# Yeicor/sdf-viewer

Hardware: AMD Instinct MI355X
Metric: Mvoxels/s grid fill + Mrays/s sphere-trace @1080p, demo SDF (higher is better)
Workload: dtype f32

## Files before the change

### include/sdfgrid.h

```cpp
#ifndef SDFGRID_H
#define SDFGRID_H

#include <stddef.h>
#include <stdint.h>

#ifdef __cplusplus
extern "C" {
#endif

#define SDFV_ABI_VERSION 5

typedef enum sdfv_status {
    SDFV_OK = 0,
    SDFV_ERR_INVALID_ARGUMENT = -1,
    SDFV_ERR_UNKNOWN_SDF = -2,
    SDFV_ERR_HIP = -3,
    SDFV_ERR_NO_DEVICE = -4,
    SDFV_ERR_COMM = -5
} sdfv_status;

typedef struct sdfv_sample {
    float distance;
    float color[3];
    float metallic;
// ... 58 lines not shown
    int32_t status;
    int32_t steps;
    float   hit_pos[3];
    float   t;
    float   raw0[4];
    float   raw1[4];
    float   normal[3];
    float   depth;
} sdfv_march_aux;

uint32_t    sdfv_abi_version(void);
const char *sdfv_last_error(void);
const char *sdfv_build_id(void);
int         sdfv_device_count(void);
float       sdfv_air_dist(void);

typedef enum sdfv_option {
    SDFV_OPT_FILL_NONTEMPORAL = 1,
    SDFV_OPT_FILL_FORM = 2,
    SDFV_OPT_RAYMARCH_DISABLE = 3,
    SDFV_OPT_RAYMARCH_KEEP_NORMAL = 4,
    SDFV_OPT_SLAB_STEP_FORM = 5,
    SDFV_OPT_RAYMARCH_TILE_GROUP = 6,
    SDFV_OPT_RAYMARCH_BOX_FIRST = 7,
    SDFV_OPT_RAYMARCH_WAVES_PER_SIMD = 8,
    SDFV_OPT_RAYMARCH_BATCH_STREAMS = 9,
    SDFV_OPT_EXT_SRGB_QUANT = 10,
    SDFV_OPT_PASS_INDEX_LIMIT = 11,
    SDFV_OPT_RAYMARCH_CAMERA_STAGING = 12,
    SDFV_OPT_PASS_FORM = 13,
    SDFV_OPT_PASS_LOADS = 15,
    SDFV_OPT_RCCL_LIBRARY = 14,
    SDFV_OPT_RAYMARCH_LOD_FILTER = 16,
    SDFV_OPT_TUNING_WAVE_TIMING = 100,
    SDFV_OPT_TUNING_TILE_ORDER = 102,
    SDFV_OPT_TUNING_PRIORITY_MAP = 101
} sdfv_option;
#define SDFV_RM_NO_FAST_INDEX  1u
#define SDFV_RM_NO_POW2_EXTENT 2u
#define SDFV_RM_NO_POW2_SIZE   4u
#define SDFV_RM_NO_SYMMETRIC   8u
#define SDFV_RM_NO_ASM_LOOP   16u
#define SDFV_RM_NO_INTERIOR_FETCH 32u
#define SDFV_STEP_SIDE_BOUNDARY 3u
#define SDFV_STEP_UNPACKED     4u
#define SDFV_STEP_START_EVENT  8u
#define SDFV_STEP_DEFER_JOIN  16u
int sdfv_set_option(uint32_t option, uint64_t value);
int sdfv_get_option(uint32_t option, uint64_t *value);

void sdfv_demo_params_default(sdfv_demo_params *p);
int  sdfv_grid_from_bb(const float bb_min[3], const float bb_max[3], uint32_t max_voxels_side, sdfv_grid *out);
void sdfv_render_params_default(sdfv_render_params *rp, const sdfv_grid *grid);
int  sdfv_camera_look_at(sdfv_camera *cam, const float eye[3], const float target[3], const float up[3],
                         float fovy_degrees, float aspect, float z_near, float z_far);


int sdfv_grid_init(const sdfv_grid *grid, float *tex0, float *tex1, void *stream);

int sdfv_grid_init_unvisited(const sdfv_grid *grid, uint32_t step, float *tex0, float *tex1, float *dist, void *stream);
int sdfv_grid_init_unvisited_ex(const sdfv_grid *grid, uint32_t step, float *tex0, float *tex1, float *dist, uint32_t flags,
                                void *stream);

int sdfv_fill_grid(const sdfv_demo_params *params, uint32_t sdf_id, const sdfv_grid *grid,
                   float *tex0, float *tex1, void *stream);

// ... 311 lines not shown
```

### sdf-viewer_amd/_capi.py

```python
import ctypes as C
import os

_HERE = os.path.dirname(os.path.abspath(__file__))
LIB_PATH = os.environ.get("SDFGRID_LIBRARY") or os.path.join(_HERE, "libsdfgrid.so")


class SdfvError(RuntimeError):
    def __init__(self, code, message):
        super().__init__(f"libsdfgrid error {code}: {message}")
        self.code = code


class Sample(C.Structure):
    _fields_ = [("distance", C.c_float), ("color", C.c_float * 3), ("metallic", C.c_float),
                ("roughness", C.c_float), ("occlusion", C.c_float)]


class DemoParams(C.Structure):
    _fields_ = [("cube_half_side", C.c_float), ("cube_material", C.c_uint32),
                ("sphere_radius", C.c_float), ("sphere_material", C.c_uint32),
                ("max_distance_custom_material", C.c_float), ("disable_sphere", C.c_uint32)]


class Grid(C.Structure):
# ... 171 lines not shown
                                            C.c_uint32, C.POINTER(Mesh), C.c_void_p]),
    "sdfv_lattice_normals": (C.c_int, [C.c_void_p, C.POINTER(C.c_float), C.POINTER(C.c_float), C.c_uint32, C.c_void_p, C.c_size_t,
                                       C.c_void_p]),
}
MESH_WITH_MATERIALS = 1
MESHER_MARCHING_CUBES = 0
MESHER_DUAL_CONTOURING_PARTICLE = 4
LIGHT_AMBIENT, LIGHT_DIRECTIONAL, MAX_LIGHTS = 0, 1, 4


def raymarch_rc(rp, tex0, tex1, cameras, n_cameras, width, height, y0, y1, rgba, depth=None, aux=None, dist=None, pairs=None,
                ilv=None, band_first=0, band_step=0, stream=None, size=None, band_height=0):
    d = MarchDesc()
    d.size = C.sizeof(d) if size is None else size
    d.rp = C.pointer(rp) if rp is not None else None
    d.tex0, d.tex1, d.dist, d.pairs, d.ilv = tex0, tex1, dist, pairs, ilv
    if cameras is not None:
        d.cameras = C.cast(C.pointer(cameras), C.POINTER(Camera))
    d.n_cameras, d.width, d.height, d.y0, d.y1 = n_cameras, width, height, y0, y1
    d.band_first, d.band_step, d.band_height = band_first, band_step, band_height
    d.rgba, d.depth, d.aux = rgba, depth, aux
    return lib.sdfv_raymarch_ex(C.byref(d), stream)
OPT_FILL_NONTEMPORAL, OPT_FILL_FORM, OPT_RAYMARCH_DISABLE, OPT_RAYMARCH_KEEP_NORMAL, OPT_SLAB_STEP_FORM = 1, 2, 3, 4, 5
OPT_RAYMARCH_TILE_GROUP = 6
OPT_RAYMARCH_BOX_FIRST = 7
OPT_RAYMARCH_WAVES_PER_SIMD = 8
OPT_RAYMARCH_BATCH_STREAMS = 9
OPT_PASS_INDEX_LIMIT = 11
OPT_RAYMARCH_CAMERA_STAGING = 12
OPT_PASS_FORM = 13
OPT_RCCL_LIBRARY = 14
OPT_PASS_LOADS = 15
OPT_RAYMARCH_LOD_FILTER = 16
OPT_EXT_SRGB_QUANT = 10
OPT_TUNING_WAVE_TIMING = 100
OPT_TUNING_PRIORITY_MAP = 101
OPT_TUNING_TILE_ORDER = 102
RM_NO_FAST_INDEX, RM_NO_POW2_EXTENT, RM_NO_POW2_SIZE, RM_NO_SYMMETRIC, RM_NO_ASM_LOOP, RM_NO_INTERIOR_FETCH = 1, 2, 4, 8, 16, 32
STEP_SIDE_BOUNDARY, STEP_UNPACKED, STEP_START_EVENT, STEP_DEFER_JOIN = 3, 4, 8, 16
PASS_FRESH_GRID, PASS_SAME_LOAD, PASS_VIRGIN_GRID, PASS_VOLUME_INTERLEAVED, PASS_EXPECT_NOOP = 1, 2, 4, 8, 16
(OP_SPHERE, OP_CUBE, OP_BOX, OP_CYLINDER, OP_TORUS, OP_PLANE, OP_PUSH_AFFINE, OP_PUSH_SCALE, OP_POP, OP_POP_SCALE, OP_UNION,
 OP_INTERSECT, OP_SUBTRACT, OP_SMOOTH_UNION, OP_SMOOTH_SUBTRACT, OP_ROUND, OP_SHELL, OP_MATERIAL) = range(1, 19)
PROGRAM_MAX_OPS, PROGRAM_MAX_VALUES, PROGRAM_MAX_FRAMES = 256, 8, 4
FILL_FORM = {"auto": 0, "rows": 1, "flat": 2}
COMM_ID_BYTES = 128
RAY_BUFFER_HEADER_BYTES = 16
MARCH_MERGE = 1
COMM_PERIODIC = 1
COMM_HALO2 = 2


def load(path=LIB_PATH):
    if not os.path.exists(path):
        raise ImportError(
            f"{path} not found: build it with `python -c 'import __graft_entry__ as g; g.build()'` "
            "(or `make -C sdf-viewer_amd/csrc`).  There is no CPU fallback.")
    lib = C.CDLL(path)
    for name, (restype, argtypes) in PROTOTYPES.items():
        fn = getattr(lib, name)
        fn.restype = restype
        fn.argtypes = argtypes
    return lib


lib = load()

# ... 9 lines not shown
```

### sdf-viewer_amd/csrc/api_common.hip

```cpp
#include <atomic>
#include <cmath>
#include <cstdarg>
#include <cstdio>
#include <cstring>
#include <mutex>
#include <string>

#include "api_internal.h"

namespace sdfv {
thread_local char g_err[512] = "";
thread_local Options g_options;

int set_error(int code, const char* fmt, ...) {
    va_list ap;
    va_start(ap, fmt);
    vsnprintf(g_err, sizeof(g_err), fmt, ap);
    va_end(ap);
    return code;
}

int hip_fail(hipError_t e, const char* what) {
    if (e == hipErrorNoDevice || e == hipErrorInvalidDevice)
        return set_error(SDFV_ERR_NO_DEVICE, "%s: no HIP device (%s)", what, hipGetErrorString(e));
// ... 112 lines not shown

int sdfv_set_option(uint32_t option, uint64_t value) {
    auto out_of_range = [&] {
        return set_error(SDFV_ERR_INVALID_ARGUMENT, "value %llu is out of range for option %u", (unsigned long long)value, option);
    };
    for (const auto& o : kPlainOptions) {
        if (o.option != option) continue;
        if (value > o.max) return out_of_range();
        g_options.*o.member = (uint32_t)value;
        return SDFV_OK;
    }
    switch (option) {
        case SDFV_OPT_SLAB_STEP_FORM: {
            const uint64_t form = value & ~(uint64_t)(SDFV_STEP_UNPACKED | SDFV_STEP_START_EVENT | SDFV_STEP_DEFER_JOIN);
            if (form != 0 && form != SDFV_STEP_SIDE_BOUNDARY) break;
            g_options.slab_step_form = (uint32_t)value;
            return SDFV_OK;
        }
        case SDFV_OPT_PASS_INDEX_LIMIT:
            if (value != 0 && (value < 2 || value > (1ull << 32))) break;
            g_options.pass_index_limit = value;
            return SDFV_OK;
        case SDFV_OPT_RCCL_LIBRARY: {
            const char* path = reinterpret_cast<const char*>((uintptr_t)value);
            if (path && strnlen(path, 4096) >= 4096) break;
            if (!sdfv::set_rccl_library_path(path))
                return set_error(SDFV_ERR_INVALID_ARGUMENT, "SDFV_OPT_RCCL_LIBRARY: RCCL has already been loaded in this process");
            return SDFV_OK;
        }
        case SDFV_OPT_RAYMARCH_WAVES_PER_SIMD:
            if (value == 1 || value > 7) break;
            g_options.raymarch_waves_per_simd = (uint32_t)value;
            return SDFV_OK;
        case SDFV_OPT_TUNING_TILE_ORDER: case SDFV_OPT_TUNING_PRIORITY_MAP: case SDFV_OPT_TUNING_WAVE_TIMING: {
#ifdef SDFV_TUNING
            (option == SDFV_OPT_TUNING_TILE_ORDER ? g_options.tile_order
             : option == SDFV_OPT_TUNING_PRIORITY_MAP ? g_options.priority_map : g_options.wave_timing) = value;
            return SDFV_OK;
#else
            const char* name = option == SDFV_OPT_TUNING_TILE_ORDER ? "TILE_ORDER" : option == SDFV_OPT_TUNING_PRIORITY_MAP ? "PRIORITY_MAP" : "WAVE_TIMING";
            return set_error(SDFV_ERR_INVALID_ARGUMENT, "SDFV_OPT_TUNING_%s needs the tuning build (make tuning)", name);
#endif
        }
        default:
            return set_error(SDFV_ERR_INVALID_ARGUMENT, "unknown option %u", option);
    }
    return out_of_range();
}

int sdfv_get_option(uint32_t option, uint64_t* value) {
    if (!value) return set_error(SDFV_ERR_INVALID_ARGUMENT, "value is NULL");
    for (const auto& o : kPlainOptions)
        if (o.option == option) {
            *value = g_options.*o.member;
            return SDFV_OK;
        }
    switch (option) {
        case SDFV_OPT_SLAB_STEP_FORM: *value = g_options.slab_step_form; return SDFV_OK;
        case SDFV_OPT_TUNING_WAVE_TIMING: *value = g_options.wave_timing; return SDFV_OK;
        case SDFV_OPT_TUNING_PRIORITY_MAP: *value = g_options.priority_map; return SDFV_OK;
        case SDFV_OPT_TUNING_TILE_ORDER: *value = g_options.tile_order; return SDFV_OK;
        case SDFV_OPT_RAYMARCH_WAVES_PER_SIMD: *value = g_options.raymarch_waves_per_simd; return SDFV_OK;
        case SDFV_OPT_PASS_INDEX_LIMIT: *value = g_options.pass_index_limit; return SDFV_OK;
        case SDFV_OPT_RCCL_LIBRARY: {
            thread_local std::string copy;
            copy = sdfv::rccl_library_path_copy();
            *value = (uint64_t)(uintptr_t)copy.c_str();
            return SDFV_OK;
        }
        default: return set_error(SDFV_ERR_INVALID_ARGUMENT, "unknown option %u", option);
    }
}

void sdfv_demo_params_default(sdfv_demo_params* p) {
    if (!p) return;
    p->cube_half_side = 0.95f;
    p->cube_material = SDFV_MATERIAL_BRICK;
    p->sphere_radius = 1.05f;
    p->sphere_material = SDFV_MATERIAL_NORMAL;
    p->max_distance_custom_material = 0.05f;
    p->disable_sphere = 0;
}

int sdfv_grid_from_bb(const float bb_min[3], const float bb_max[3], uint32_t max_voxels_side, sdfv_grid* out) {
    if (!bb_min || !bb_max || !out) return set_error(SDFV_ERR_INVALID_ARGUMENT, "NULL argument");
    float size[3] = {bb_max[0] - bb_min[0], bb_max[1] - bb_min[1], bb_max[2] - bb_min[2]};
    int max_dim = 0;
    for (int i = 1; i < 3; ++i)
        if (size[i] >= size[max_dim]) max_dim = i;
    for (int i = 0; i < 3; ++i) {
        if (i == max_dim) {
            out->dims[i] = max_voxels_side;
        } else {
            float v = (float)max_voxels_side * size[i] / size[max_dim];
            out->dims[i] = v > 0.0f ? (uint32_t)v : 0u;
// ... 53 lines not shown
```

### sdf-viewer_amd/csrc/api_internal.h

```cpp
#pragma once

#include <hip/hip_runtime.h>

#include <cstdint>
#include <cstring>
#include <string>

#include "../../include/sdfgrid.h"

namespace sdfv {
struct Options {
    uint32_t fill_nontemporal = 0;
    uint32_t fill_form = 0;
    uint32_t raymarch_disable = 0;
    uint32_t raymarch_keep_normal = 0;
    uint32_t raymarch_lod_filter = 0;
    uint32_t raymarch_batch_streams = 1;
    uint32_t raymarch_camera_staging = 1;
    uint32_t raymarch_box_first = 1;
    uint32_t raymarch_waves_per_simd = 0;
    uint32_t raymarch_tile_group = 0;
    uint32_t slab_step_form = 0;
    uint32_t ext_srgb_quant = 0;
    uint32_t pass_form = 0;
    uint32_t pass_loads = 0;
    unsigned long long pass_index_limit = 0;
    unsigned long long wave_timing = 0;
    unsigned long long priority_map = 0;
    unsigned long long tile_order = 0;
};
extern thread_local char g_err[512];
extern thread_local Options g_options;
inline const Options& options() { return g_options; }
std::string rccl_library_path_copy();
const char* claim_rccl_library_path();
int set_error(int code, const char* fmt, ...) __attribute__((format(printf, 2, 3)));
int hip_fail(hipError_t e, const char* what);
#define SDFV_HIP(call)                                          \
    do {                                                        \
        hipError_t e_ = (call);                                 \
        if (e_ != hipSuccess) return sdfv::hip_fail(e_, #call); \
    } while (0)
#define SDFV_HIP_RETURN(call) return sdfv::hip_status((call), #call)
inline int hip_status(hipError_t e, const char* what) { return e == hipSuccess ? SDFV_OK : hip_fail(e, what); }

int check_params(const sdfv_demo_params* p, uint32_t sdf_id);
int check_grid(const sdfv_grid* g);
int check_lights(const sdfv_render_params* rp);
int need_device();
inline int need_textures(const void* tex0, const void* tex1) {
    return tex0 && tex1 ? SDFV_OK : set_error(SDFV_ERR_INVALID_ARGUMENT, "texture pointer is NULL");
}
template <typename... P>
// ... 96 lines not shown
```

### sdf-viewer_amd/csrc/api_march.hip

```cpp
#include <cmath>
#include <cstddef>
#include <cstring>

#include "api_internal.h"
#include "march_common.h"
#include "raymarch_kernels.h"

using namespace sdfv;

namespace {

struct BatchStreams {
    static constexpr int kSide = 3;
    hipStream_t side[kSide] = {};
    hipEvent_t fork = nullptr, join[kSide] = {};
    int device = -1;
    void release() {
        for (int i = 0; i < kSide; ++i) {
            if (side[i]) (void)hipStreamDestroy(side[i]);
            if (join[i]) (void)hipEventDestroy(join[i]);
        }
        if (fork) (void)hipEventDestroy(fork);
        *this = BatchStreams{};
    }
// ... 118 lines not shown
    if (int rc = check_lights(rp)) return rc;
    if (int rc = check_texel_alignment(d.tex0, d.tex1, d.rgba)) return rc;
    if (int rc = check_word_aligned("dist, depth, aux and rgba8", d.dist, d.depth, d.aux, d.rgba8)) return rc;
    if (((uintptr_t)d.pairs | (uintptr_t)d.ilv) & 7) return set_error(SDFV_ERR_INVALID_ARGUMENT, "pairs and ilv must be 8-byte aligned");
    if (n_cameras && !cameras) return set_error(SDFV_ERR_INVALID_ARGUMENT, "cameras is NULL");
    if (y0 > y1 || y1 > height) return set_error(SDFV_ERR_INVALID_ARGUMENT, "rows [%u,%u) outside height %u", y0, y1, height);
    if (rp->tex_size[0] == 0 || rp->tex_size[1] == 0 || rp->tex_size[2] == 0)
        return set_error(SDFV_ERR_INVALID_ARGUMENT, "empty texture");
    if (!(rp->lod_dist_between_samples >= 1.0f)) return set_error(SDFV_ERR_INVALID_ARGUMENT, "lod_dist_between_samples < 1");
    const uint32_t lod_filter = g_options.raymarch_lod_filter;
    if (lod_filter == 1 && rp->lod_dist_between_samples != 1.0f) {
        int e = 0;
        const float lod = rp->lod_dist_between_samples;
        if (!(lod >= 2.0f && lod <= 32768.0f) || frexpf(lod, &e) != 0.5f)
            return set_error(SDFV_ERR_INVALID_ARGUMENT,
                             "SDFV_OPT_RAYMARCH_LOD_FILTER 1: lod_dist_between_samples %g is not a power of two in [2, 32768]", (double)lod);
    }
    if ((uint64_t)rp->tex_size[0] * rp->tex_size[1] * rp->tex_size[2] >= (1ull << 32))
        return set_error(SDFV_ERR_INVALID_ARGUMENT, "texture too large for 32-bit texel indexing");
    if (int rc = need_device()) return rc;
    sdfv::RaymarchArgs a;
    derive_raymarch_args(rp, a);
    a.dist = d.dist;
    a.pairs = d.pairs;
    a.ilv = d.ilv;
    set_march_frame(a, d.tex0, d.tex1, width, height, y0, y1);
    a.band_skip = band_height * (band_step - 1u);
    a.band_shift = band_height == 8u ? 3u : 4u;
    a.rows_out = band_step > 1 ? sdfv_band_rows_ex(height, y0 / band_height, band_step, band_height) : y1 - y0;
    a.compute_normal = g_options.raymarch_keep_normal ? 1u : 0u;
    const uint32_t w = g_options.raymarch_waves_per_simd;
    a.waves_per_simd = w;
    a.box_first = g_options.raymarch_box_first;
    const DeviceFacts& dev = device_facts();
    if (!dev.gfx950) a.asm_loop = 0;
    a.wave_slots_per_simd_unit = dev.cus * 4u;
    a.last_level_cache_bytes = dev.last_level_cache_bytes;
    const bool xcd_order_ok = dev.xcds == 8;
    a.group_shift = g_options.raymarch_tile_group == 0 ? (n_cameras == 1 && xcd_order_ok ? sdfv::kGroupAuto : 0u)
                                                       : (g_options.raymarch_tile_group == 1 ? 0u : g_options.raymarch_tile_group - 1u);
    a.rotate_columns = g_options.raymarch_tile_group == 0 && xcd_order_ok ? 1u : 0u;
#ifdef SDFV_TUNING
    a.wave_timing = reinterpret_cast<unsigned long long*>(g_options.wave_timing);
    a.priority_map = reinterpret_cast<const unsigned char*>(g_options.priority_map);
    a.tile_order = n_cameras == 1 ? reinterpret_cast<const uint32_t*>(g_options.tile_order) : nullptr;
#endif
    const uint64_t pixels_per_cam = (uint64_t)a.rows_out * width;
    hipStream_t main = (hipStream_t)stream;
    const sdfv_camera* device_cameras = nullptr;
    bool ring = false;
    hipPointerAttribute_t attr;
    if (hipPointerGetAttributes(&attr, cameras) == hipSuccess && (attr.type == hipMemoryTypeDevice || attr.type == hipMemoryTypeManaged)) {
        device_cameras = cameras;
    } else {
        (void)hipGetLastError();
        if (n_cameras > sdfv::kInlineCameras) {
            hipStreamCaptureStatus capturing = hipStreamCaptureStatusNone;
            if (hipStreamIsCapturing(main, &capturing) != hipSuccess) (void)hipGetLastError();
            ring = capturing == hipStreamCaptureStatusNone && g_options.raymarch_camera_staging &&
                   g_camera_ring.ensure(current_device()) == hipSuccess;
        }
    }
    const uint32_t per_launch = device_cameras || ring ? sdfv::kMaxCamerasPerLaunch : sdfv::kInlineCameras;
    const uint64_t groups_per_launch = (uint64_t)((width + 15) / 16) * ((a.rows_out + 15) / 16) * per_launch;
    const bool overlap = n_cameras > per_launch && groups_per_launch <= 40000 && g_options.raymarch_batch_streams;
    uint32_t used = 0;
// ... 217 lines not shown
```

### sdf-viewer_amd/csrc/march_common.h

```cpp
#pragma once

#include "march_shade.h"

#if defined(__HIPCC__)
#define SDFV_MARCH_FN __device__ __forceinline__
#define SDFV_MARCH_HD __host__ __device__ __forceinline__
#else
#define SDFV_MARCH_FN inline
#define SDFV_MARCH_HD inline
#endif

namespace sdfv {
namespace march {

struct V3 {
    float x, y, z;
};
SDFV_MARCH_FN V3 mk(float x, float y, float z) { V3 r; r.x = x; r.y = y; r.z = z; return r; }
SDFV_MARCH_FN V3 sub(V3 a, V3 b) { return mk(a.x - b.x, a.y - b.y, a.z - b.z); }
SDFV_MARCH_FN V3 madd(V3 a, V3 d, float t) { return mk(a.x + d.x * t, a.y + d.y * t, a.z + d.z * t); }
SDFV_MARCH_FN float length(V3 a) { return sqrtf(a.x * a.x + a.y * a.y + a.z * a.z); }
SDFV_MARCH_FN V3 normalize(V3 a) {
    const float l = length(a);
    return mk(a.x / l, a.y / l, a.z / l);
// ... 42 lines not shown
}
SDFV_MARCH_FN V3 tap_sign(int t) { return mk((t == 0 || t == 3) ? 1.0f : -1.0f, t >= 2 ? 1.0f : -1.0f, (t & 1) ? 1.0f : -1.0f); }
SDFV_MARCH_FN V3 normal_tap(V3 p, float h, int t) {
    const V3 k = tap_sign(t);
    return mk(p.x + k.x * h, p.y + k.y * h, p.z + k.z * h);
}
SDFV_MARCH_FN V3 normal_of_taps(float d1, float d2, float d3, float d4) {
    return normalize(mk(d1 + -d2 + -d3 + d4, -d1 + -d2 + d3 + d4, -d1 + d2 + -d3 + d4));
}

SDFV_MARCH_FN void aux_clear(sdfv_march_aux& aux) {
    aux.status = 0; aux.steps = 0;
    aux.hit_pos[0] = aux.hit_pos[1] = aux.hit_pos[2] = 0.0f;
    aux.t = 0.0f;
    aux.raw0[0] = aux.raw0[1] = aux.raw0[2] = aux.raw0[3] = 0.0f;
    aux.raw1[0] = aux.raw1[1] = aux.raw1[2] = aux.raw1[3] = 0.0f;
    aux.normal[0] = aux.normal[1] = aux.normal[2] = 0.0f;
    aux.depth = 1.0f;
}
SDFV_MARCH_FN void aux_set_march(sdfv_march_aux& aux, int status, int steps, V3 ray_pos, float dist_from_origin) {
    aux.status = status;
    aux.steps = steps;
    aux.hit_pos[0] = ray_pos.x; aux.hit_pos[1] = ray_pos.y; aux.hit_pos[2] = ray_pos.z;
    aux.t = dist_from_origin;
}
SDFV_MARCH_FN void aux_set_hit(sdfv_march_aux& aux, float4 raw0, float4 raw1, V3 n, float depth) {
    aux.raw0[0] = raw0.x; aux.raw0[1] = raw0.y; aux.raw0[2] = raw0.z; aux.raw0[3] = raw0.w;
    aux.raw1[0] = raw1.x; aux.raw1[1] = raw1.y; aux.raw1[2] = raw1.z; aux.raw1[3] = raw1.w;
    aux.normal[0] = n.x; aux.normal[1] = n.y; aux.normal[2] = n.z;
    aux.depth = depth;
}

#if defined(__HIPCC__)
SDFV_MARCH_FN void tile_pixel(uint32_t bx, uint32_t by, uint32_t& px, uint32_t& row) {
    const uint32_t lane = threadIdx.x & 63, wave = threadIdx.x >> 6;
    px = bx * 16 + (wave & 1) * 8 + (lane & 7);
    row = by * 16 + (wave >> 1) * 8 + (lane >> 3);
}

template <typename Args>
SDFV_MARCH_FN void store_color(const Args& a, uint64_t out_index, float4 v) {
    typedef float v4f __attribute__((ext_vector_type(4)));
    if (a.rgba) {
        const v4f t = {v.x, v.y, v.z, v.w};
        __builtin_nontemporal_store(t, reinterpret_cast<v4f*>(a.rgba + out_index));
    }
    if (a.rgba8) __builtin_nontemporal_store(rgba_unorm8(v), a.rgba8 + out_index);
}
#endif

}
}
```

### sdf-viewer_amd/csrc/program_march_kernels.hip

```cpp
#include "program_march_kernels.h"

#include "kernel_common.h"

namespace sdfv {

namespace {

template <bool AUX>
__device__ __forceinline__ void program_march(const ProgramMarchArgs& a) {
    __shared__ float s_lut[256];
    const LdsLut lut = stage_srgb_lut(s_lut);
    __syncthreads();

    uint32_t px, row;
    march::tile_pixel(blockIdx.x, blockIdx.y, px, row);
    const uint32_t py = a.y0 + row;
    const uint32_t cam_idx = blockIdx.z;
    const bool in_image = px < a.f.width && py < a.y1;
    const sdfv_camera& cam = a.cameras[cam_idx];
    const uint64_t out_index = ((uint64_t)cam_idx * (a.y1 - a.y0) + row) * a.f.width + px;

    float4 rgba;
    sdfv_march_aux aux;
    pmarch::march_pixel_program(a.f, cam, px, py, in_image, lut, rgba, aux);
    if (!in_image) return;
    march::store_color(a, out_index, rgba);
    if (a.depth) a.depth[out_index] = aux.depth;
    if (AUX) a.aux[out_index] = aux;
}

}

extern "C" {

__global__ __launch_bounds__(kBlock) void sdfprog_march(ProgramMarchArgs a) { program_march<false>(a); }
__global__ __launch_bounds__(kBlock) void sdfprog_march_aux(ProgramMarchArgs a) { program_march<true>(a); }

}

hipError_t launch_program_march(const ProgramMarchArgs& a, hipStream_t stream) {
    if (a.f.width == 0 || a.y1 <= a.y0 || a.n_cameras == 0) return hipSuccess;
    if (a.n_cameras > kProgramMarchCameras) return hipErrorInvalidValue;
    const uint32_t tiles_x = (a.f.width + 15) / 16, tiles_y = (a.y1 - a.y0 + 15) / 16;
    if (tiles_y > 65535u) return hipErrorInvalidValue;
    hipLaunchKernelGGL(a.aux ? sdfprog_march_aux : sdfprog_march, dim3(tiles_x, tiles_y, a.n_cameras), dim3(kBlock), 0, stream, a);
    return hipGetLastError();
}

// ... 2 lines not shown
```

### sdf-viewer_amd/csrc/raymarch_kernels.h

```cpp
#pragma once

#include <hip/hip_runtime.h>
#include <stdint.h>

#include "../../include/sdfgrid.h"

namespace sdfv {

struct RaymarchArgs {
    sdfv_render_params rp;
    float bsize[3];
    float inv_bsize[3];
    uint32_t pow2_extent;
    uint32_t fast_index;
    const float* dist;
    const float* pairs;
    const float* ilv;
    uint32_t pow2_size;
    uint32_t symmetric_box;
    uint32_t fast_normal;
    float cull_center[3];
    float cull_radius2;
    const float4* tex0;
    const float4* tex1;
    uint32_t n_cameras;
    uint32_t width, height;
    uint32_t y0, y1;
    uint32_t compute_normal;
    uint32_t asm_loop;
    uint32_t group_shift;
    uint32_t tiles_x, tiles_y, groups_x;
    uint32_t box_first;
    uint32_t first_gx0, first_gy0, first_w, first_h, m_groups_x, m_first_w, m_rest_w;
    uint32_t no_interior_fetch;
    uint32_t rotate_columns;
    uint32_t lds_cap_bytes;
    uint32_t waves_per_simd;
    uint32_t wave_slots_per_simd_unit;
    uint64_t last_level_cache_bytes;
    uint32_t cube_box;
    uint32_t rows_out;
    uint32_t band_skip;
    uint32_t band_shift;
    float4* rgba;
    uint32_t* rgba8;
    sdfv_march_aux* aux;
    float* depth;
#ifdef SDFV_TUNING
    const uint32_t* tile_order;
    const unsigned char* priority_map;
    unsigned long long* wave_timing;
#endif
    const sdfv_camera* camera_list;
    sdfv_camera cameras[16];
};

constexpr int kMarchGeneral = 0, kMarchTex0 = 1, kMarchDist = 2, kMarchPairs = 3, kMarchIlv = 4, kMarchLattice = 5;

constexpr uint32_t kInlineCameras = 16;
constexpr uint32_t kMaxCamerasPerLaunch = 64;
constexpr uint32_t kGroupAuto = 255;

struct SlabMarchArgs {
    uint32_t z_lo, z_count;
    uint32_t own_begin, own_end;
    const sdfv_ray_state* in;
    uint32_t n_in;
    const uint32_t* in_count[2];
    const sdfv_ray_state* in_rays[2];
    uint32_t max_in;
// ... 17 lines not shown
```

### sdf-viewer_amd/csrc/raymarch_kernels.hip

```cpp
#include "raymarch_kernels.h"

#include <hip/hip_runtime.h>
#include <string.h>

#include "march_common.h"

namespace sdfv {
namespace {

using namespace march;

__device__ __forceinline__ uint32_t mirror_index(int i, int n) {
    if (i >= 0 && i < n) return (uint32_t)i;
    int period = 2 * n;
    int m = i % period;
    if (m < 0) m += period;
    return (uint32_t)(m < n ? m : period - 1 - m);
}

struct Tex {
    const float4* data;
    int w, h, d;
    int z_lo;
};
// ... 546 lines not shown
#define SDFV_MARCH_ASM_PER_VOLUME(RUN)                                                                              \
    if (MODE == kMarchIlv) { SDFV_MARCH_ASM_PER_BOX(RUN, SDFV_MARCH_ASM_VOL_ILV); }                                 \
    else if (MODE == kMarchPairs) { SDFV_MARCH_ASM_PER_BOX(RUN, SDFV_MARCH_ASM_VOL_PAIRS); }                        \
    else if (MODE == kMarchDist) { SDFV_MARCH_ASM_PER_BOX(RUN, SDFV_MARCH_ASM_VOL_DIST); }                          \
    else { SDFV_MARCH_ASM_PER_BOX(RUN, SDFV_MARCH_ASM_VOL_TEX0); }
    const bool cube = a.cube_box != 0;
    if (T) {
        float tt = dist_from_origin;
        int n = 0;
        SDFV_MARCH_ASM_PER_VOLUME(SDFV_MARCH_ASM_RUN_AUX)
        dist_from_origin = tt;
        steps = n;
    } else {
        SDFV_MARCH_ASM_PER_VOLUME(SDFV_MARCH_ASM_RUN)
    }
#ifdef SDFV_TUNING
    iterations = cov ? (min(255, 255 - (int)(short)(left & 0xffff)) | (left & 0xffff0000)) : 0;
#else
    (void)iterations;
    (void)left;
#endif
    if (covered) {
        ray_pos = mk(px, py, pz);
        const bool ran = ((ran_out >> (threadIdx.x & 63)) & 1ull) != 0;
        status = ran ? -1 : (oob_dist<true>(a, ray_pos) > 1e-4f ? -2 : 1);
    }
}

#ifdef SDFV_TUNING
__device__ __forceinline__ void stamp_wave(const RaymarchArgs& a, uint32_t bx, uint32_t by, uint32_t wave,
                                           unsigned long long t_start, unsigned long long t_start_rt, int iterations,
                                           unsigned long long covered_mask) {
    const uint32_t tiles_x = (a.width + 15) / 16, tiles_y = (a.rows_out + 15) / 16;
    const uint64_t wave_id = ((uint64_t)(blockIdx.z * tiles_y + by) * tiles_x + bx) * 4 + wave;
    a.wave_timing[wave_id * 4 + 0] = t_start;
    a.wave_timing[wave_id * 4 + 1] = __builtin_readcyclecounter();
    a.wave_timing[wave_id * 4 + 2] = (unsigned long long)(uint32_t)iterations | ((t_start_rt & 0xffffull) << 32) |
                                     ((__builtin_amdgcn_s_memrealtime() & 0xffffull) << 48);
    a.wave_timing[wave_id * 4 + 3] = covered_mask;
}
#endif

__device__ __forceinline__ bool box_fragment_ray(const RaymarchArgs& a, V3 eye, V3 d_raw, bool in_image,
                                                 V3& ray_origin, V3& ray_dir) {
    const V3 d0 = normalize(d_raw);
    float tfrag;
    const bool covered = box_slab_test(a.rp, eye, d0, in_image, tfrag);
    fragment_ray(a.rp, eye, d0, tfrag, ray_origin, ray_dir);
    return covered;
}

#ifndef SDFV_RM_MIN_WAVES
#define SDFV_RM_MIN_WAVES 1
#endif
template <int MODE, bool LINEAR, int XF, bool SYMM, bool AUX, bool ASM = false, bool NORMAL = AUX>
__global__ __launch_bounds__(256, SDFV_RM_MIN_WAVES) void raymarch_kernel(RaymarchArgs a) {
    constexpr bool FAST = MODE != 0;
    static_assert(NORMAL || !AUX, "the aux record carries the normal");
#ifdef SDFV_TUNING
    const uint32_t lane = threadIdx.x & 63, wave = threadIdx.x >> 6;
#endif
    uint32_t bx = blockIdx.x, by = blockIdx.y;
#ifdef SDFV_TUNING
    if (a.tile_order) {
        const uint32_t tiles_x = (a.width + 15) / 16, t = a.tile_order[blockIdx.x];
        bx = t % tiles_x;
        by = t / tiles_x;
    } else
#endif
    if (a.group_shift == 0 && a.rotate_columns) {
        const uint32_t tiles_x = gridDim.x;
        const uint32_t r = (blockIdx.y + blockIdx.z) % tiles_x;
        bx = blockIdx.x + r;
        if (bx >= tiles_x) bx -= tiles_x;
    } else if (a.group_shift) {
        const uint32_t g = a.group_shift, per = 1u << (2 * g);
        const uint32_t L = blockIdx.x, xcd = L & 7u, k = L >> 3;
        const uint32_t G = (k >> (2 * g)) * 8u + xcd, t = k & (per - 1u);
        uint32_t gx, gy;
        if (a.first_w == 0) {
            gx = G % a.groups_x;
            gy = G / a.groups_x;
        } else {
            auto div = [](uint32_t n, uint32_t d, uint32_t m) { return d == 1 ? n : __umulhi(n, m); };
            const uint32_t n_in = a.first_w * a.first_h, top = a.first_gy0 * a.groups_x, rest_w = a.groups_x - a.first_w;
            uint32_t j = G - n_in;
            if (G < n_in) {
                const uint32_t r = div(G, a.first_w, a.m_first_w);
                gx = a.first_gx0 + (G - r * a.first_w);
                gy = a.first_gy0 + r;
            } else if (j < top) {
                gy = div(j, a.groups_x, a.m_groups_x);
                gx = j - gy * a.groups_x;
            } else if ((j -= top) < a.first_h * rest_w) {
                const uint32_t r = div(j, rest_w, a.m_rest_w), c = j - r * rest_w;
                gy = a.first_gy0 + r;
                gx = c < a.first_gx0 ? c : c + a.first_w;
            } else {
                j -= a.first_h * rest_w;
                const uint32_t r = div(j, a.groups_x, a.m_groups_x);
                gy = a.first_gy0 + a.first_h + r;
                gx = j - r * a.groups_x;
            }
        }
        bx = (gx << g) + (t & ((1u << g) - 1u));
        by = (gy << g) + (t >> g);
        if (bx >= a.tiles_x || by >= a.tiles_y) return;
    }
    uint32_t px, row;
    tile_pixel(bx, by, px, row);
    const uint32_t py = a.y0 + row + (row >> a.band_shift) * a.band_skip;
    const uint32_t cam_idx = blockIdx.z;
    const bool in_image = px < a.width && py < a.y1;
    sdfv_camera cam;
    if (a.camera_list) cam = a.camera_list[cam_idx];
    else cam = a.cameras[cam_idx];
    const uint64_t out_index = ((uint64_t)cam_idx * a.rows_out + row) * a.width + px;
#ifdef SDFV_TUNING
    if (a.priority_map && a.priority_map[by * ((a.width + 15) / 16) + bx]) __builtin_amdgcn_s_setprio(3);
    const unsigned long long t_start = a.wave_timing ? __builtin_readcyclecounter() : 0ull;
    const unsigned long long t_start_rt = a.wave_timing ? __builtin_amdgcn_s_memrealtime() : 0ull;
#endif

    const V3 eye = mk(cam.eye[0], cam.eye[1], cam.eye[2]);
    const V3 d_raw = pixel_ray_raw(a.width, a.height, cam, px, py);

    {
        const V3 m = sub(eye, mk(a.cull_center[0], a.cull_center[1], a.cull_center[2]));
        const float dd = d_raw.x * d_raw.x + d_raw.y * d_raw.y + d_raw.z * d_raw.z;
        const float mm = m.x * m.x + m.y * m.y + m.z * m.z;
        const float md = m.x * d_raw.x + m.y * d_raw.y + m.z * d_raw.z;
        const float r2 = a.cull_radius2;
        const bool miss = mm > r2 && (md >= 0.0f || mm * dd - md * md > r2 * dd);
        if (__ballot(in_image && !miss) == 0ull) {
            if (in_image) {
                store_color(a, out_index, make_float4(0.0f, 0.0f, 0.0f, 0.0f));
                if (AUX) {
                    sdfv_march_aux aux;
                    aux_clear(aux);
                    a.aux[out_index] = aux;
                }
            }
            if (in_image && a.depth) a.depth[out_index] = 1.0f;
// ... 363 lines not shown
    } else {
        if (a.aux) hipLaunchKernelGGL((raymarch_slab_kernel<0, true>), grid, dim3(256), 0, stream, a, s);
        else hipLaunchKernelGGL((raymarch_slab_kernel<0, false>), grid, dim3(256), 0, stream, a, s);
    }
    return hipGetLastError();
}

namespace {

int march_volume_mode(const RaymarchArgs& a) { return march_volume_choice(a, a.dist != nullptr, a.pairs != nullptr, a.ilv != nullptr); }

struct MarchKernel {
    int mode;
    bool linear;
    int xf;
    bool symm;
    bool hand_written_loop;
};

MarchKernel select_march_kernel(const RaymarchArgs& a, uint32_t lod_filter) {
    MarchKernel k{kMarchGeneral, a.rp.lod_dist_between_samples == 1.0f, a.pow2_extent ? 1 : 0, false, false};
    if (!k.linear && lod_filter == 1) k.mode = kMarchLattice;
    if (!k.linear || !a.fast_index) return k;
    k.mode = march_volume_mode(a);
    if (k.mode == 0) k.mode = a.dist ? kMarchDist : kMarchTex0;
    if (a.pow2_extent && a.pow2_size) k.xf = 2;
    k.symm = k.xf >= 1 && a.symmetric_box;
    k.hand_written_loop = hand_written_loop_applies(a) && volume_fits_loop(a, k.mode);
    return k;
}

template <int MODE, bool LINEAR, int XF, bool SYMM, bool ASM>
void launch_variant(const RaymarchArgs& a, dim3 grid, hipStream_t stream) {
    if (a.aux)
        hipLaunchKernelGGL((raymarch_kernel<MODE, LINEAR, XF, SYMM, true, ASM>), grid, dim3(256), a.lds_cap_bytes, stream, a);
    else if (a.compute_normal)
        hipLaunchKernelGGL((raymarch_kernel<MODE, LINEAR, XF, SYMM, false, ASM, true>), grid, dim3(256), a.lds_cap_bytes, stream, a);
    else
        hipLaunchKernelGGL((raymarch_kernel<MODE, LINEAR, XF, SYMM, false, ASM>), grid, dim3(256), a.lds_cap_bytes, stream, a);
}

constexpr int variant_key(int mode, bool linear, int xf, bool symm, bool hand_written_loop) {
    return mode | (linear ? 8 : 0) | (xf << 4) | (symm ? 64 : 0) | (hand_written_loop ? 128 : 0);
}

hipError_t launch_selected(const MarchKernel& k, const RaymarchArgs& a, dim3 grid, hipStream_t stream) {
#define SDFV_VARIANT(MODE, LINEAR, XF, SYMM, ASM) \
    case variant_key(MODE, LINEAR, XF, SYMM, ASM): launch_variant<MODE, LINEAR, XF, SYMM, ASM>(a, grid, stream); break
    switch (variant_key(k.mode, k.linear, k.xf, k.symm, k.hand_written_loop)) {
        SDFV_VARIANT(kMarchIlv, true, 2, true, true);
        SDFV_VARIANT(kMarchPairs, true, 2, true, true);
        SDFV_VARIANT(kMarchDist, true, 2, true, true);
        SDFV_VARIANT(kMarchDist, true, 2, true, false);
        SDFV_VARIANT(kMarchDist, true, 2, false, false);
        SDFV_VARIANT(kMarchDist, true, 1, true, false);
        SDFV_VARIANT(kMarchDist, true, 1, false, false);
        SDFV_VARIANT(kMarchDist, true, 0, false, false);
        SDFV_VARIANT(kMarchTex0, true, 2, true, true);
        SDFV_VARIANT(kMarchTex0, true, 2, true, false);
        SDFV_VARIANT(kMarchTex0, true, 2, false, false);
        SDFV_VARIANT(kMarchTex0, true, 1, true, false);
        SDFV_VARIANT(kMarchTex0, true, 1, false, false);
        SDFV_VARIANT(kMarchTex0, true, 0, false, false);
        SDFV_VARIANT(kMarchGeneral, true, 1, false, false);
        SDFV_VARIANT(kMarchGeneral, true, 0, false, false);
        SDFV_VARIANT(kMarchGeneral, false, 1, false, false);
        SDFV_VARIANT(kMarchGeneral, false, 0, false, false);
        SDFV_VARIANT(kMarchLattice, false, 1, false, false);
        SDFV_VARIANT(kMarchLattice, false, 0, false, false);
    default: return hipErrorInvalidValue;
    }
#undef SDFV_VARIANT
// ... 16 lines not shown
        const float px = (xc / (zc * cam.aspect * cam.tan_half_fovy) + 1.0f) * 0.5f * (float)ag.width;
        const float py = (1.0f - yc / (zc * cam.tan_half_fovy)) * 0.5f * (float)ag.height - (float)ag.y0;
        if (!(px == px) || !(py == py)) return;
        x_lo = fminf(x_lo, px), x_hi = fmaxf(x_hi, px), y_lo = fminf(y_lo, py), y_hi = fmaxf(y_hi, py);
    }
    const float edge = (float)(16u << ag.group_shift), gxs = (float)ag.groups_x, gys = (float)groups_y;
    const float fx0 = fminf(fmaxf(floorf((x_lo - 1.0f) / edge), 0.0f), gxs), fx1 = fminf(fmaxf(floorf((x_hi + 1.0f) / edge) + 1.0f, 0.0f), gxs);
    const float fy0 = fminf(fmaxf(floorf((y_lo - 1.0f) / edge), 0.0f), gys), fy1 = fminf(fmaxf(floorf((y_hi + 1.0f) / edge) + 1.0f, 0.0f), gys);
    if (!(fx1 > fx0) || !(fy1 > fy0)) return;
    ag.first_gx0 = (uint32_t)fx0, ag.first_gy0 = (uint32_t)fy0;
    ag.first_w = (uint32_t)(fx1 - fx0), ag.first_h = (uint32_t)(fy1 - fy0);
    if (ag.first_w == ag.groups_x && ag.first_h == groups_y) {
        ag.first_w = 0;
        return;
    }
    auto magic = [](uint32_t d) { return d <= 1 ? 0u : (uint32_t)(((1ull << 32) + d - 1) / d); };
    ag.m_groups_x = magic(ag.groups_x), ag.m_first_w = magic(ag.first_w), ag.m_rest_w = magic(ag.groups_x - ag.first_w);
}

static uint32_t occupancy_rule(const RaymarchArgs& ag) {
    if (ag.waves_per_simd >= 2 && ag.waves_per_simd <= 6) return ag.waves_per_simd;
    if (ag.waves_per_simd == 7) return 7;
    if (ag.n_cameras != 1 || ag.first_w == 0 || ag.group_shift == 0 || ag.wave_slots_per_simd_unit == 0) return 7;
    const uint64_t texels = (uint64_t)ag.rp.tex_size[0] * ag.rp.tex_size[1] * ag.rp.tex_size[2];
    const int mode = march_volume_mode(ag);
    const uint64_t volume_bytes = texels * (mode == kMarchPairs ? 8u : ((mode == kMarchIlv || ag.dist) ? 4u : 16u));
    if (ag.last_level_cache_bytes == 0 || volume_bytes <= ag.last_level_cache_bytes) return 7;
    const uint64_t rect_waves = (uint64_t)ag.first_w * ag.first_h * (4ull << (2 * ag.group_shift));
    const uint64_t slots7 = 7ull * ag.wave_slots_per_simd_unit;
    if (rect_waves < slots7 || 2 * rect_waves > 7 * slots7) return 7;
    return 4;
}

static uint32_t lds_cap_for(uint32_t w) {
    uint32_t bytes = (w >= 2 && w <= 6) ? (160u * 1024u) / w - 1024u : 0u;
    if (bytes > 65536u) bytes = 65536u;
    return bytes;
}

hipError_t launch_raymarch(const RaymarchArgs& a, hipStream_t stream, uint32_t lod_filter) {
    const uint32_t rows = a.rows_out;
    if (a.width == 0 || rows == 0 || a.n_cameras == 0) return hipSuccess;
    dim3 grid((a.width + 15) / 16, (rows + 15) / 16, a.n_cameras);
    RaymarchArgs ag = a;
    const dim3 tiles = grid;
#ifdef SDFV_TUNING
    if (a.tile_order) {
        ag.group_shift = 0;
        ag.lds_cap_bytes = lds_cap_for(occupancy_rule(ag));
        return launch_selected(select_march_kernel(ag, lod_filter), ag, dim3(tiles.x * tiles.y, 1, 1), stream);
    }
#endif
    auto grouped = [&](uint32_t shift) {
        ag.group_shift = shift;
        ag.tiles_x = tiles.x;
        ag.tiles_y = tiles.y;
        ag.groups_x = (tiles.x + (1u << shift) - 1) >> shift;
        const uint32_t groups_y = (tiles.y + (1u << shift) - 1) >> shift;
        const uint32_t groups = ((ag.groups_x * groups_y + 7u) / 8u) * 8u;
        ag.first_w = 0;
        if (a.box_first && a.n_cameras == 1 && groups < 65536u) box_first_rectangle(ag, groups_y);
        grid = dim3(groups << (2 * shift), 1, a.n_cameras);
    };
    if (a.band_skip) {
        ag.group_shift = 0;
    } else if (a.group_shift == kGroupAuto) {
        grouped(1);
        if (ag.first_w == 0) grouped(2);
    } else if (a.group_shift) {
        grouped(a.group_shift);
    }
    ag.lds_cap_bytes = lds_cap_for(occupancy_rule(ag));
    return launch_selected(select_march_kernel(ag, lod_filter), ag, grid, stream);
}

}
```

Baseline: 203,700.

## Allow single- or two-wave raymarch workgroups with matching tile mapping and LDS cap

Measured after the change: 204,000 (median of 3 runs). Within noise of the previous version (+0.1%).

```diff
diff --git a/include/sdfgrid.h b/include/sdfgrid.h
--- a/include/sdfgrid.h
+++ b/include/sdfgrid.h
@@ -114,6 +114,7 @@
     SDFV_OPT_PASS_LOADS = 15,
     SDFV_OPT_RCCL_LIBRARY = 14,
     SDFV_OPT_RAYMARCH_LOD_FILTER = 16,
+    SDFV_OPT_RAYMARCH_WORKGROUP_WAVES = 17,
     SDFV_OPT_TUNING_WAVE_TIMING = 100,
     SDFV_OPT_TUNING_TILE_ORDER = 102,
     SDFV_OPT_TUNING_PRIORITY_MAP = 101
diff --git a/sdf-viewer_amd/_capi.py b/sdf-viewer_amd/_capi.py
--- a/sdf-viewer_amd/_capi.py
+++ b/sdf-viewer_amd/_capi.py
@@ -227,6 +227,7 @@
 OPT_RCCL_LIBRARY = 14
 OPT_PASS_LOADS = 15
 OPT_RAYMARCH_LOD_FILTER = 16
+OPT_RAYMARCH_WORKGROUP_WAVES = 17
 OPT_EXT_SRGB_QUANT = 10
 OPT_TUNING_WAVE_TIMING = 100
 OPT_TUNING_PRIORITY_MAP = 101
diff --git a/sdf-viewer_amd/csrc/api_common.hip b/sdf-viewer_amd/csrc/api_common.hip
--- a/sdf-viewer_amd/csrc/api_common.hip
+++ b/sdf-viewer_amd/csrc/api_common.hip
@@ -168,6 +168,10 @@
             if (value == 1 || value > 7) break;
             g_options.raymarch_waves_per_simd = (uint32_t)value;
             return SDFV_OK;
+        case SDFV_OPT_RAYMARCH_WORKGROUP_WAVES:
+            if (value != 0 && value != 1 && value != 2 && value != 4) break;
+            g_options.raymarch_workgroup_waves = (uint32_t)value;
+            return SDFV_OK;
         case SDFV_OPT_TUNING_TILE_ORDER: case SDFV_OPT_TUNING_PRIORITY_MAP: case SDFV_OPT_TUNING_WAVE_TIMING: {
 #ifdef SDFV_TUNING
             (option == SDFV_OPT_TUNING_TILE_ORDER ? g_options.tile_order
@@ -197,6 +201,7 @@
         case SDFV_OPT_TUNING_PRIORITY_MAP: *value = g_options.priority_map; return SDFV_OK;
         case SDFV_OPT_TUNING_TILE_ORDER: *value = g_options.tile_order; return SDFV_OK;
         case SDFV_OPT_RAYMARCH_WAVES_PER_SIMD: *value = g_options.raymarch_waves_per_simd; return SDFV_OK;
+        case SDFV_OPT_RAYMARCH_WORKGROUP_WAVES: *value = g_options.raymarch_workgroup_waves; return SDFV_OK;
         case SDFV_OPT_PASS_INDEX_LIMIT: *value = g_options.pass_index_limit; return SDFV_OK;
         case SDFV_OPT_RCCL_LIBRARY: {
             thread_local std::string copy;
diff --git a/sdf-viewer_amd/csrc/api_internal.h b/sdf-viewer_amd/csrc/api_internal.h
--- a/sdf-viewer_amd/csrc/api_internal.h
+++ b/sdf-viewer_amd/csrc/api_internal.h
@@ -19,6 +19,7 @@
     uint32_t raymarch_camera_staging = 1;
     uint32_t raymarch_box_first = 1;
     uint32_t raymarch_waves_per_simd = 0;
+    uint32_t raymarch_workgroup_waves = 0;
     uint32_t raymarch_tile_group = 0;
     uint32_t slab_step_form = 0;
     uint32_t ext_srgb_quant = 0;
diff --git a/sdf-viewer_amd/csrc/api_march.hip b/sdf-viewer_amd/csrc/api_march.hip
--- a/sdf-viewer_amd/csrc/api_march.hip
+++ b/sdf-viewer_amd/csrc/api_march.hip
@@ -174,6 +174,7 @@
     const uint32_t w = g_options.raymarch_waves_per_simd;
     a.waves_per_simd = w;
     a.box_first = g_options.raymarch_box_first;
+    a.workgroup_waves = g_options.raymarch_workgroup_waves;
     const DeviceFacts& dev = device_facts();
     if (!dev.gfx950) a.asm_loop = 0;
     a.wave_slots_per_simd_unit = dev.cus * 4u;
diff --git a/sdf-viewer_amd/csrc/march_common.h b/sdf-viewer_amd/csrc/march_common.h
--- a/sdf-viewer_amd/csrc/march_common.h
+++ b/sdf-viewer_amd/csrc/march_common.h
@@ -98,10 +98,10 @@
 }
 
 #if defined(__HIPCC__)
-SDFV_MARCH_FN void tile_pixel(uint32_t bx, uint32_t by, uint32_t& px, uint32_t& row) {
+SDFV_MARCH_FN void tile_pixel(uint32_t bx, uint32_t by, uint32_t sx, uint32_t sy, uint32_t& px, uint32_t& row) {
     const uint32_t lane = threadIdx.x & 63, wave = threadIdx.x >> 6;
-    px = bx * 16 + (wave & 1) * 8 + (lane & 7);
-    row = by * 16 + (wave >> 1) * 8 + (lane >> 3);
+    px = ((bx << sx) + (wave & ((1u << sx) - 1u))) * 8 + (lane & 7);
+    row = ((by << sy) + (wave >> sx)) * 8 + (lane >> 3);
 }
 
 template <typename Args>
diff --git a/sdf-viewer_amd/csrc/program_march_kernels.hip b/sdf-viewer_amd/csrc/program_march_kernels.hip
--- a/sdf-viewer_amd/csrc/program_march_kernels.hip
+++ b/sdf-viewer_amd/csrc/program_march_kernels.hip
@@ -13,7 +13,7 @@
     __syncthreads();
 
     uint32_t px, row;
-    march::tile_pixel(blockIdx.x, blockIdx.y, px, row);
+    march::tile_pixel(blockIdx.x, blockIdx.y, 1, 1, px, row);
     const uint32_t py = a.y0 + row;
     const uint32_t cam_idx = blockIdx.z;
     const bool in_image = px < a.f.width && py < a.y1;
diff --git a/sdf-viewer_amd/csrc/raymarch_kernels.h b/sdf-viewer_amd/csrc/raymarch_kernels.h
--- a/sdf-viewer_amd/csrc/raymarch_kernels.h
+++ b/sdf-viewer_amd/csrc/raymarch_kernels.h
@@ -36,6 +36,8 @@
     uint32_t rotate_columns;
     uint32_t lds_cap_bytes;
     uint32_t waves_per_simd;
+    uint32_t workgroup_waves;
+    uint32_t wg_shift_x, wg_shift_y;
     uint32_t wave_slots_per_simd_unit;
     uint64_t last_level_cache_bytes;
     uint32_t cube_box;
diff --git a/sdf-viewer_amd/csrc/raymarch_kernels.hip b/sdf-viewer_amd/csrc/raymarch_kernels.hip
--- a/sdf-viewer_amd/csrc/raymarch_kernels.hip
+++ b/sdf-viewer_amd/csrc/raymarch_kernels.hip
@@ -602,12 +602,16 @@
                                            unsigned long long t_start, unsigned long long t_start_rt, int iterations,
                                            unsigned long long covered_mask) {
     const uint32_t tiles_x = (a.width + 15) / 16, tiles_y = (a.rows_out + 15) / 16;
-    const uint64_t wave_id = ((uint64_t)(blockIdx.z * tiles_y + by) * tiles_x + bx) * 4 + wave;
+    const uint32_t wx = (bx << a.wg_shift_x) + (wave & ((1u << a.wg_shift_x) - 1u)), wy = (by << a.wg_shift_y) + (wave >> a.wg_shift_x);
+    const uint64_t wave_id = ((uint64_t)(blockIdx.z * tiles_y + (wy >> 1)) * tiles_x + (wx >> 1)) * 4 + ((wy & 1) * 2 + (wx & 1));
     a.wave_timing[wave_id * 4 + 0] = t_start;
     a.wave_timing[wave_id * 4 + 1] = __builtin_readcyclecounter();
     a.wave_timing[wave_id * 4 + 2] = (unsigned long long)(uint32_t)iterations | ((t_start_rt & 0xffffull) << 32) |
                                      ((__builtin_amdgcn_s_memrealtime() & 0xffffull) << 48);
-    a.wave_timing[wave_id * 4 + 3] = covered_mask;
+    const uint32_t hw_id = __builtin_amdgcn_s_getreg(4 | (31 << 11)), xcc_id = __builtin_amdgcn_s_getreg(20 | (31 << 11));
+    const unsigned long long place = ((hw_id >> 4) & 3u) | (((hw_id >> 8) & 0xffu) << 2) | ((xcc_id & 0xfu) << 10);
+    const unsigned long long setup = covered_mask & 0xffffffffull;
+    a.wave_timing[wave_id * 4 + 3] = (setup < 0x3ffffull ? setup : 0x3ffffull) | (place << 18) | (covered_mask & 0xffffffff00000000ull);
 }
 #endif
 
@@ -644,9 +648,9 @@
         bx = blockIdx.x + r;
         if (bx >= tiles_x) bx -= tiles_x;
     } else if (a.group_shift) {
-        const uint32_t g = a.group_shift, per = 1u << (2 * g);
+        const uint32_t gsx = a.group_shift + 1u - a.wg_shift_x, gsy = a.group_shift + 1u - a.wg_shift_y;
         const uint32_t L = blockIdx.x, xcd = L & 7u, k = L >> 3;
-        const uint32_t G = (k >> (2 * g)) * 8u + xcd, t = k & (per - 1u);
+        const uint32_t G = (k >> (gsx + gsy)) * 8u + xcd, t = k & ((1u << (gsx + gsy)) - 1u);
         uint32_t gx, gy;
         if (a.first_w == 0) {
             gx = G % a.groups_x;
@@ -673,12 +677,12 @@
                 gx = j - r * a.groups_x;
             }
         }
-        bx = (gx << g) + (t & ((1u << g) - 1u));
-        by = (gy << g) + (t >> g);
+        bx = (gx << gsx) + (t & ((1u << gsx) - 1u));
+        by = (gy << gsy) + (t >> gsx);
         if (bx >= a.tiles_x || by >= a.tiles_y) return;
     }
     uint32_t px, row;
-    tile_pixel(bx, by, px, row);
+    tile_pixel(bx, by, a.wg_shift_x, a.wg_shift_y, px, row);
     const uint32_t py = a.y0 + row + (row >> a.band_shift) * a.band_skip;
     const uint32_t cam_idx = blockIdx.z;
     const bool in_image = px < a.width && py < a.y1;
@@ -1108,12 +1112,13 @@
 
 template <int MODE, bool LINEAR, int XF, bool SYMM, bool ASM>
 void launch_variant(const RaymarchArgs& a, dim3 grid, hipStream_t stream) {
+    const dim3 block(64u << (a.wg_shift_x + a.wg_shift_y));
     if (a.aux)
-        hipLaunchKernelGGL((raymarch_kernel<MODE, LINEAR, XF, SYMM, true, ASM>), grid, dim3(256), a.lds_cap_bytes, stream, a);
+        hipLaunchKernelGGL((raymarch_kernel<MODE, LINEAR, XF, SYMM, true, ASM>), grid, block, a.lds_cap_bytes, stream, a);
     else if (a.compute_normal)
-        hipLaunchKernelGGL((raymarch_kernel<MODE, LINEAR, XF, SYMM, false, ASM, true>), grid, dim3(256), a.lds_cap_bytes, stream, a);
+        hipLaunchKernelGGL((raymarch_kernel<MODE, LINEAR, XF, SYMM, false, ASM, true>), grid, block, a.lds_cap_bytes, stream, a);
     else
-        hipLaunchKernelGGL((raymarch_kernel<MODE, LINEAR, XF, SYMM, false, ASM>), grid, dim3(256), a.lds_cap_bytes, stream, a);
+        hipLaunchKernelGGL((raymarch_kernel<MODE, LINEAR, XF, SYMM, false, ASM>), grid, block, a.lds_cap_bytes, stream, a);
 }
 
 constexpr int variant_key(int mode, bool linear, int xf, bool symm, bool hand_written_loop) {
@@ -1196,10 +1201,22 @@
     return 4;
 }
 
-static uint32_t lds_cap_for(uint32_t w) {
-    uint32_t bytes = (w >= 2 && w <= 6) ? (160u * 1024u) / w - 1024u : 0u;
+static uint32_t lds_cap_for(uint32_t w, uint32_t workgroup_waves) {
+    if (w < 2 || w > 6) return 0u;
+    uint32_t bytes = (128u / (4u * w / workgroup_waves)) * 1280u;
     if (bytes > 65536u) bytes = 65536u;
     return bytes;
+}
+
+static uint32_t workgroup_rule(const RaymarchArgs& ag, uint32_t cap) {
+    if (ag.n_cameras != 1 || ag.group_shift == 0) return 4;
+#ifdef SDFV_TUNING
+    if (ag.priority_map) return 4;
+#endif
+    uint32_t waves = ag.workgroup_waves;
+    if (waves == 0) waves = ag.first_w != 0 ? 1 : 4;
+    if (waves == 1 && (cap == 5 || cap == 6)) waves = 2;
+    return waves;
 }
 
 hipError_t launch_raymarch(const RaymarchArgs& a, hipStream_t stream, uint32_t lod_filter) {
@@ -1207,24 +1224,23 @@
     if (a.width == 0 || rows == 0 || a.n_cameras == 0) return hipSuccess;
     dim3 grid((a.width + 15) / 16, (rows + 15) / 16, a.n_cameras);
     RaymarchArgs ag = a;
+    ag.wg_shift_x = ag.wg_shift_y = 1;
     const dim3 tiles = grid;
 #ifdef SDFV_TUNING
     if (a.tile_order) {
         ag.group_shift = 0;
-        ag.lds_cap_bytes = lds_cap_for(occupancy_rule(ag));
+        ag.lds_cap_bytes = lds_cap_for(occupancy_rule(ag), 4);
         return launch_selected(select_march_kernel(ag, lod_filter), ag, dim3(tiles.x * tiles.y, 1, 1), stream);
     }
 #endif
+    uint32_t groups = 0;
     auto grouped = [&](uint32_t shift) {
         ag.group_shift = shift;
-        ag.tiles_x = tiles.x;
-        ag.tiles_y = tiles.y;
         ag.groups_x = (tiles.x + (1u << shift) - 1) >> shift;
         const uint32_t groups_y = (tiles.y + (1u << shift) - 1) >> shift;
-        const uint32_t groups = ((ag.groups_x * groups_y + 7u) / 8u) * 8u;
+        groups = ((ag.groups_x * groups_y + 7u) / 8u) * 8u;
         ag.first_w = 0;
         if (a.box_first && a.n_cameras == 1 && groups < 65536u) box_first_rectangle(ag, groups_y);
-        grid = dim3(groups << (2 * shift), 1, a.n_cameras);
     };
     if (a.band_skip) {
         ag.group_shift = 0;
@@ -1234,7 +1250,15 @@
     } else if (a.group_shift) {
         grouped(a.group_shift);
     }
-    ag.lds_cap_bytes = lds_cap_for(occupancy_rule(ag));
+    const uint32_t cap = occupancy_rule(ag), waves = workgroup_rule(ag, cap);
+    ag.wg_shift_x = waves >= 2 ? 1 : 0;
+    ag.wg_shift_y = waves == 4 ? 1 : 0;
+    if (ag.group_shift) {
+        ag.tiles_x = (a.width + (8u << ag.wg_shift_x) - 1) / (8u << ag.wg_shift_x);
+        ag.tiles_y = (rows + (8u << ag.wg_shift_y) - 1) / (8u << ag.wg_shift_y);
+        grid = dim3(groups << (2 * ag.group_shift + 2 - ag.wg_shift_x - ag.wg_shift_y), 1, a.n_cameras);
+    }
+    ag.lds_cap_bytes = lds_cap_for(cap, waves);
     return launch_selected(select_march_kernel(ag, lod_filter), ag, grid, stream);
 }
 
```
